# AnirudhKaushik10/Efficient-Workers-in-Distributed-Machine-Learning

Hardware: AMD Instinct MI355X
Metric: grad bytes/step on wire + images/sec, VGG-11 CIFAR-10 at 1/2/4/8 MI355X (higher is better)
Workload: dtype fp32

## Files before the change

efficient-workers-in-distributed-machine-learning_amd/ops/csrc/bindings.cpp:

```cpp
#include <pybind11/pybind11.h>
#include <pybind11/stl.h>

#include <vector>

#include "ewdml_ops.h"

namespace py = pybind11;
using Ptrs = std::vector<uintptr_t>;
using Mask = std::vector<uint32_t>;

static GradSrc grad_src(const Ptrs& grads, const Mask& mask) {
  return GradSrc{grads.data(), (int)grads.size(), mask.data(), (int)mask.size()};
}

template <class A, void (*fn)(const A&)>
static void with_grads(A a, const Ptrs& grads, const Mask& mask) {
  a.src = grad_src(grads, mask);
  fn(a);
}

static StepArgs default_step() {
  StepArgs s{};
  s.grad_scale = 1.0f;
  return s;
// ... 233 lines not shown
  m.def("cf_flush_wgout", &ew_cf_flush_wgout);
  m.def("bn_part_floats", &ew_bn_part_floats);
  m.def("bn_relu_fwd",
        [](uintptr_t h, uintptr_t res, uintptr_t y, uintptr_t code, uintptr_t stats,
           uintptr_t part, uintptr_t gamma, uintptr_t beta, uintptr_t cbias, uintptr_t rmean,
           uintptr_t rvar, uintptr_t nbt, long long N, int H, int W, int C, int is_bf16,
           int pool, int mode, int training, float momentum, float eps, int cb_bf16,
           uintptr_t stream, int pre_nblk, int phase) {
          BnFwdArgs a{};
          a.pre_nblk = pre_nblk;
          a.phase = phase;
          a.h = h; a.res = res; a.y = y; a.code = code; a.stats = stats; a.part = part;
          a.gamma = gamma; a.beta = beta; a.cbias = cbias; a.rmean = rmean; a.rvar = rvar;
          a.nbt = nbt; a.N = N; a.H = H; a.W = W; a.C = C;
          a.is_bf16 = is_bf16; a.pool = pool; a.mode = mode; a.training = training;
          a.momentum = momentum; a.eps = eps; a.cb_bf16 = cb_bf16; a.stream = stream;
          ew_bn_relu_fwd(a);
        });
  m.def("bn_relu_bwd",
        [](uintptr_t h, uintptr_t res, uintptr_t dy, uintptr_t code, uintptr_t stats,
           uintptr_t coef, uintptr_t part, uintptr_t dx, uintptr_t dres, uintptr_t dgamma,
           uintptr_t dbeta, uintptr_t dcbias, long long N, int H, int W, int C, int is_bf16,
           int pool, int mode, int cb_bf16, uintptr_t stream, int pre_nblk, int phase) {
          BnBwdArgs a{};
          a.phase = phase;
          a.h = h; a.res = res; a.dy = dy; a.code = code; a.stats = stats; a.coef = coef;
          a.part = part; a.dx = dx; a.dres = dres; a.dgamma = dgamma; a.dbeta = dbeta;
          a.dcbias = dcbias; a.N = N; a.H = H; a.W = W; a.C = C; a.is_bf16 = is_bf16;
          a.pool = pool; a.mode = mode; a.cb_bf16 = cb_bf16; a.stream = stream;
          a.pre_nblk = pre_nblk;
          ew_bn_relu_bwd(a);
        });
  m.def("act_dropout_fwd", &ew_act_dropout_fwd);
  m.def("act_dropout_bwd", &ew_act_dropout_bwd);
  m.def("cross_entropy_fwd", &ew_cross_entropy_fwd);
  m.def("cross_entropy_bwd", &ew_cross_entropy_bwd);
  m.def("conv_ws_floats", &ew_conv_ws_floats);
  m.def("conv_fwd", &ew_conv_fwd);
  m.def("conv_bwd_data", &ew_conv_bwd_data);
  m.def("conv_wgrad", &ew_conv_wgrad);
  m.def("conv_stem_fwd", &ew_conv_stem_fwd);
  m.def("head_fwd", &ew_head_fwd);
  m.def("head_fwd_ce", &ew_head_fwd_ce);
  m.def("head_bwd", &ew_head_bwd);
  m.def("head_bwd_bn", &ew_head_bwd_bn);
  m.def("conv_stem_wgrad", &ew_conv_stem_wgrad);
  m.def("rccl_unique_id", [] { return pybind11::bytes(ew_rccl_unique_id()); });
  m.def("rccl_version", &ew_rccl_version);
  m.def("rccl_init", [](pybind11::bytes uid, int nranks, int rank, int device) {
    return ew_rccl_init(std::string(uid), nranks, rank, device);
  });
  m.def("rccl_destroy", &ew_rccl_destroy);
  m.def("rccl_abort", &ew_rccl_abort);
  m.def("rccl_watchdog_start", &ew_rccl_watchdog_start);
  m.def("rccl_watch", &ew_rccl_watch);
  m.def("rccl_watch_pending", &ew_rccl_watch_pending);
  m.def("rccl_watchdog_stop", &ew_rccl_watchdog_stop,
        pybind11::call_guard<pybind11::gil_scoped_release>());
  m.def("test_flag_alloc", &ew_test_flag_alloc);
  m.def("test_flag_free", &ew_test_flag_free);
  m.def("watchdog_release_flag", &ew_watchdog_release_flag);
  m.def("test_spin", &ew_test_spin);
  m.def("rccl_all_gather", &ew_rccl_all_gather);
  m.def("rccl_all_reduce", &ew_rccl_all_reduce);
  m.def("rccl_reduce_scatter", &ew_rccl_reduce_scatter);
  m.def("rccl_broadcast", &ew_rccl_broadcast);
  m.def("rccl_all_to_all", &ew_rccl_all_to_all);
  m.def("conv_f32_fwd", &ew_conv_f32_fwd);
  m.def("conv_f32_bwd_data", &ew_conv_f32_bwd_data);
  m.def("conv_f32_wgrad", &ew_conv_f32_wgrad);
  m.def("conv_f32_fwd_lz", &ew_conv_f32_fwd_lz);
  m.def("conv_f32_wgrad_lz", &ew_conv_f32_wgrad_lz);
  m.def("conv_f32_fwd_s2", &ew_conv_f32_fwd_s2);
  m.def("conv_f32_bwd_data_s2", &ew_conv_f32_bwd_data_s2);
  m.def("conv_f32_wgrad_s2", &ew_conv_f32_wgrad_s2);
  m.def("conv_f32_stem_fwd", &ew_conv_f32_stem_fwd);
  m.def("conv_f32_stem_wgrad", &ew_conv_f32_stem_wgrad);
  m.def("conv_f32_stem_wgrad_bn", &ew_conv_f32_stem_wgrad_bn);
  m.def("wino_f32_weight", &ew_wino_f32_weight);
  m.def("wino_f32_fwd", &ew_wino_f32_fwd);
  m.def("wino_f32_bwd_data", &ew_wino_f32_bwd_data);
  m.def("wino_f32_wgrad", &ew_wino_f32_wgrad);
  m.def("wino_f32_wgrad_out", &ew_wino_f32_wgrad_out);
  m.def("wino_f32_fwd_bn", &ew_wino_f32_fwd_bn);
  m.def("wino_f32_bwd_data_bn", &ew_wino_f32_bwd_data_bn);
  m.def("sm_f32_ws_floats", &ew_sm_f32_ws_floats);
  m.def("sm_f32_counters", &ew_sm_f32_counters);
  m.def("sm_f32_fwd", &ew_sm_f32_fwd);
  m.def("sm_set_fence", &ew_sm_set_fence);
  m.def("topk_fused_select_max_blocks", &ew_topk_fused_select_max_blocks);
  m.def("topk_one_max_blocks", &ew_topk_one_max_blocks);
  m.def("flag_signal", &ew_flag_signal);
  m.def("flag_wait", &ew_flag_wait);
  m.def("topk_one_stamps", &ew_topk_one_stamps);
  m.def("sm_f32_bwd", &ew_sm_f32_bwd);
  m.def("lenet_ws_floats", &ew_lenet_ws_floats);
  m.def("lenet_counters", &ew_lenet_counters);
  m.def("lenet_set_prof", &ew_lenet_set_prof);
  m.def("lenet_fwd", &ew_lenet_fwd);
  m.def("tail_ws_floats", &ew_tail_ws_floats);
  m.def("tail_counters", &ew_tail_counters);
  m.def("tail_fwd", &ew_tail_fwd);
  m.def("tail_bwd", &ew_tail_bwd);
  m.def("lenet_bwd", &ew_lenet_bwd);
  m.def("maxpool2_nhwc", &ew_maxpool2_nhwc);
  m.def("maxpool3s2_nhwc", &ew_maxpool3s2_nhwc);
  m.def("gap_nhwc", &ew_gap_nhwc);
  m.def("maxpool2_fwd", &ew_maxpool2_fwd);
  m.def("maxpool2_bwd", &ew_maxpool2_bwd);
  m.def("ticket_ints", [] { return EW_TICKET_INTS; });
  m.def("make_batch",
        [](uintptr_t src, uintptr_t labels, uintptr_t perm, long long perm_len, uintptr_t state,
           uintptr_t done, uintptr_t out, uintptr_t out_y, int B, int C, int H, int W, int pad, int augment,
           int out_bf16, int channels_last, uint32_t seed, uint32_t rank,
           const std::vector<float>& mean, const std::vector<float>& inv_std, uintptr_t stream) {
          MakeBatchArgs a{};
          a.src = src; a.labels = labels; a.perm = perm; a.perm_len = perm_len; a.state = state; a.done = done;
          a.out = out; a.out_y = out_y; a.B = B; a.C = C; a.H = H; a.W = W; a.pad = pad;
          a.augment = augment; a.out_bf16 = out_bf16; a.channels_last = channels_last;
          a.seed = seed; a.rank = rank;
          for (int c = 0; c < 4; ++c) {
            a.mean[c] = c < (int)mean.size() ? mean[c] : 0.0f;
            a.inv_std[c] = c < (int)inv_std.size() ? inv_std[c] : 1.0f;
          }
          a.stream = stream;
          ew_make_batch(a);
        });
}
```

efficient-workers-in-distributed-machine-learning_amd/ops/csrc/ewdml_ops.h:

```cpp
#pragma once
#include <stdexcept>
#include <string>
#include <vector>
#include <stddef.h>
#include <stdint.h>

struct GradSrc {
  const uintptr_t* grad_ptrs;
  int n_grad_ptrs;
  const uint32_t* bf16_mask;
  int n_bf16_mask;
};

struct StepArgs {
  uintptr_t param, mom, grad_out, shadow;
  float lr, momentum, dampening, weight_decay, grad_scale;
  int nesterov, first, apply;
  uintptr_t key_state;
  uint32_t key_seed, key_rank;
  uintptr_t lr_ptr;
};

inline void ew_step_check(const std::string& who, const StepArgs& s, bool need_mom) {
  if (s.apply && !s.param) throw std::runtime_error(who + ": apply needs the parameters");
// ... 467 lines not shown
void ew_head_fwd(uintptr_t x, uintptr_t w, uintptr_t b, uintptr_t z, uintptr_t y, int B, int N,
                 int K, int relu, uintptr_t ctr_in, uint32_t salt_in, float p_in,
                 uintptr_t ctr_out, uint32_t salt_out, float p_out, uintptr_t stream,
                 int is_f32);
void ew_head_fwd_ce(uintptr_t x, uintptr_t w, uintptr_t b, uintptr_t z, int B, int N, int K,
                    uintptr_t yl, uintptr_t lossrow, uintptr_t loss, uintptr_t lse, uintptr_t dlog,
                    uintptr_t tick, uintptr_t stream, int is_f32);
void ew_head_bwd_bn(uintptr_t dz, uintptr_t y, uintptr_t x, uintptr_t w, uintptr_t dx,
                    uintptr_t dw, uintptr_t db, int B, int N, int K, int relu, uintptr_t ctr_out,
                    uint32_t salt_out, float p_out, uintptr_t ctr_in, uint32_t salt_in,
                    float p_in, int advance, uintptr_t bn_h, uintptr_t bn_code,
                    uintptr_t bn_stats, uintptr_t bn_coef, uintptr_t bn_dgamma,
                    uintptr_t bn_dbeta, uintptr_t bn_dcbias, int bn_cb_bf16, uintptr_t bn_tick,
                    uintptr_t stream);
void ew_head_bwd(uintptr_t dz, uintptr_t y, uintptr_t x, uintptr_t w, uintptr_t dx, uintptr_t dw,
                 uintptr_t db, int db_bf16, int B, int N, int K, int relu, uintptr_t ctr_out,
                 uint32_t salt_out, float p_out, uintptr_t ctr_in, uint32_t salt_in, float p_in,
                 int advance, uintptr_t stream, int is_f32);
int ew_conv_stem_fwd(uintptr_t x, uintptr_t w, uintptr_t y, long long N, int H, int W, int Nc,
                     uintptr_t bnpart, long long bnpart_floats, uintptr_t stream);
void ew_conv_stem_wgrad(uintptr_t dy, uintptr_t x, uintptr_t dw, uintptr_t ws,
                        long long ws_floats, long long N, int H, int W, int Nc, uintptr_t stream);

int ew_conv_f32_fwd(uintptr_t x, uintptr_t w, uintptr_t y, uintptr_t ws, long long ws_floats,
                    long long N, int H, int W, int C, int Nc, int ksize, uintptr_t bnpart,
                    long long bnpart_floats, uintptr_t stream);
int ew_conv_f32_bwd_data(uintptr_t dy, uintptr_t w, uintptr_t dx, uintptr_t ws,
                         long long ws_floats, long long N, int H, int W, int C, int Nc, int ksize,
                         uintptr_t bn_h, uintptr_t bn_res, uintptr_t bn_code, uintptr_t bn_stats,
                         int bn_relu, uintptr_t bnpart, long long bnpart_floats, uintptr_t addend,
                         uintptr_t stream);
void ew_conv_f32_wgrad(uintptr_t dy, uintptr_t x, uintptr_t dw, uintptr_t ws, long long ws_floats,
                       long long N, int H, int W, int C, int Nc, int ksize, uintptr_t stream);
int ew_conv_f32_fwd_lz(uintptr_t h, uintptr_t stats, uintptr_t nbt, uintptr_t w, uintptr_t y,
                       uintptr_t ws, long long ws_floats, long long N, int H, int W, int C, int Nc,
                       uintptr_t bnpart, long long bnpart_floats, uintptr_t stream);
void ew_conv_f32_wgrad_lz(uintptr_t dy, uintptr_t h, uintptr_t stats, uintptr_t dw, uintptr_t ws,
                          long long ws_floats, long long N, int H, int W, int C, int Nc,
                          uintptr_t stream);
int ew_conv_f32_fwd_s2(uintptr_t x, uintptr_t w, uintptr_t y, uintptr_t ws, long long ws_floats,
                       long long N, int H, int W, int C, int Nc, int ksize, uintptr_t bnpart,
                       long long bnpart_floats, uintptr_t stream);
void ew_conv_f32_bwd_data_s2(uintptr_t dy, uintptr_t w, uintptr_t dx, long long N, int H, int W,
                             int C, int Nc, int ksize, uintptr_t addend, uintptr_t stream);
void ew_conv_f32_wgrad_s2(uintptr_t dy, uintptr_t x, uintptr_t dw, uintptr_t ws,
                          long long ws_floats, long long N, int H, int W, int C, int Nc, int ksize,
                          uintptr_t stream);
int ew_conv_f32_stem_fwd(uintptr_t x, uintptr_t w, uintptr_t y, long long N, int H, int W, int Nc,
                         uintptr_t bnpart, long long bnpart_floats, uintptr_t stream);
void ew_conv_f32_stem_wgrad(uintptr_t dy, uintptr_t x, uintptr_t dw, uintptr_t ws,
                            long long ws_floats, long long N, int H, int W, int Nc,
                            uintptr_t stream);
void ew_conv_f32_stem_wgrad_bn(uintptr_t h, uintptr_t dnext, uintptr_t code, uintptr_t stats,
                               uintptr_t coef, int pool, uintptr_t x, uintptr_t dw, uintptr_t ws,
                               long long ws_floats, long long N, int H, int W, int Nc,
                               uintptr_t stream);
void ew_wino_f32_weight(uintptr_t w, uintptr_t U, int Nc, int C, int m, uintptr_t stream);
int ew_wino_f32_fwd(uintptr_t x, uintptr_t w, uintptr_t U, uintptr_t y, uintptr_t V, uintptr_t Mo,
                    long long N, int H, int W, int C, int Nc, int m, uintptr_t bnpart,
                    long long bnpart_floats, uintptr_t stream);
int ew_wino_f32_bwd_data(uintptr_t dy, uintptr_t w, uintptr_t U, uintptr_t dx, uintptr_t V,
                         uintptr_t Mo, long long N, int H, int W, int C, int Nc, int m,
                         uintptr_t bn_h, uintptr_t bn_res, uintptr_t bn_code, uintptr_t bn_stats,
                         int bn_relu, uintptr_t bnpart, long long bnpart_floats,
                         uintptr_t addend, uintptr_t D, uintptr_t wo_src, int wo_split,
                         uintptr_t wo_dw, int wo_Nc, int wo_C, uintptr_t stream);
int ew_wino_f32_fwd_bn(uintptr_t bn_h, uintptr_t bn_stats, uintptr_t bn_code, uintptr_t nbt,
                       int pool, uintptr_t w, uintptr_t U, uintptr_t y, uintptr_t V,
                       uintptr_t Mo, long long N, int H, int W, int C, int Nc, int m,
                       uintptr_t bnpart, long long bnpart_floats, uintptr_t stream);
int ew_wino_f32_bwd_data_bn(uintptr_t out_h, uintptr_t out_dnext, uintptr_t out_code,
                            uintptr_t out_stats, uintptr_t out_coef, int out_pool, uintptr_t w,
                            uintptr_t U, uintptr_t dx, uintptr_t V, uintptr_t Mo, long long N,
                            int H, int W, int C, int Nc, int m, uintptr_t bn_h, uintptr_t bn_res,
                            uintptr_t bn_code, uintptr_t bn_stats, int bn_relu, uintptr_t bnpart,
                            long long bnpart_floats, uintptr_t addend, uintptr_t D,
                            uintptr_t wo_src, int wo_split, uintptr_t wo_dw, int wo_Nc, int wo_C,
                            uintptr_t stream);
int ew_wino_f32_wgrad(uintptr_t dy, uintptr_t V, uintptr_t dw, uintptr_t D, int d_ready,
                      uintptr_t U_scratch, uintptr_t ws, long long ws_floats, long long N, int H,
                      int W, int C, int Nc, int m, int defer_out, uintptr_t stream);
void ew_wino_f32_wgrad_out(uintptr_t src, int split, uintptr_t dw, int Nc, int C, int m,
                           uintptr_t stream);

long long ew_sm_f32_ws_floats(long long N, int C, int Nc);
int ew_sm_set_fence(int on);
long long ew_sm_f32_counters(long long N, int C, int Nc);
int ew_sm_f32_fwd(uintptr_t x, uintptr_t bn_h, uintptr_t bn_stats, uintptr_t nbt, uintptr_t w,
                  uintptr_t y, uintptr_t slab, long long slab_floats, uintptr_t cnt,
                  long long cnt_ints, long long N, int C, int Nc, uintptr_t bnpart,
                  long long bnpart_floats, uintptr_t stream);
int ew_sm_f32_bwd(uintptr_t x, uintptr_t bn_h, uintptr_t bn_stats, uintptr_t dy,
                  uintptr_t out_h, uintptr_t out_dnext, uintptr_t out_code, uintptr_t out_stats,
                  uintptr_t out_coef, int out_pool, uintptr_t w, uintptr_t dx, uintptr_t dw,
                  uintptr_t slab, long long slab_floats, uintptr_t cnt, long long cnt_ints,
                  long long N, int C, int Nc, uintptr_t pb_h, uintptr_t pb_res, uintptr_t pb_code,
                  uintptr_t pb_stats, int pb_relu, uintptr_t bnpart, long long bnpart_floats,
                  uintptr_t fin_coef, uintptr_t fin_dgamma, uintptr_t fin_dbeta,
                  uintptr_t fin_dcbias, int fin_cb_bf16, long long fin_M, uintptr_t stream,
                  uintptr_t st_vel = 0, uintptr_t st_resid = 0, uintptr_t st_param = 0,
                  float st_momentum = 0.0f, float st_damp1 = 1.0f, float st_wd = 0.0f,
                  int st_nesterov = 0, uintptr_t st_lr = 0, uintptr_t st_stamp = 0);

long long ew_lenet_ws_floats(int B);
int ew_lenet_counters(int B);
void ew_lenet_set_prof(uintptr_t buf);
void ew_lenet_fwd(uintptr_t x, uintptr_t w1, uintptr_t b1, uintptr_t w2, uintptr_t b2,
                  uintptr_t wf1, uintptr_t bf1, uintptr_t wf2, uintptr_t bf2, uintptr_t y, int B,
                  int K, uintptr_t a1, uintptr_t code1, uintptr_t a2, uintptr_t code2,
                  uintptr_t h1, uintptr_t logits, uintptr_t dlogits, uintptr_t dh1,
                  uintptr_t lossrow, uintptr_t loss, uintptr_t ws, long long ws_floats,
                  uintptr_t cnt, int cnt_ints, uintptr_t stream, uintptr_t bsrc = 0,
                  uintptr_t blabels = 0, uintptr_t bperm = 0, long long bperm_len = 0,
                  uintptr_t bstate = 0, uintptr_t bdone = 0, float bmean = 0.0f,
                  float binv_std = 1.0f);
void ew_lenet_bwd(uintptr_t x, uintptr_t w2, uintptr_t wf1, uintptr_t a1, uintptr_t code1,
                  uintptr_t a2, uintptr_t code2, uintptr_t h1, uintptr_t dlogits, uintptr_t dh1,
                  uintptr_t gscale, int B, int K, uintptr_t dp2, uintptr_t dw1, uintptr_t db1,
                  uintptr_t dw2, uintptr_t db2, uintptr_t dwf1, uintptr_t dbf1, uintptr_t dwf2,
                  uintptr_t dbf2, uintptr_t ws, long long ws_floats, uintptr_t cnt, int cnt_ints,
                  uintptr_t stream);

long long ew_tail_ws_floats(int B, int N2);
int ew_tail_counters(int B);
void ew_tail_fwd(uintptr_t h1, uintptr_t w2, uintptr_t b2, uintptr_t w3, uintptr_t b3, uintptr_t y,
                 int B, int K1, int N2, int K, uintptr_t h2, uintptr_t logits, uintptr_t dlogits,
                 uintptr_t dh2, uintptr_t lossrow, uintptr_t loss, uintptr_t ws,
                 long long ws_floats, uintptr_t cnt, int cnt_ints, uintptr_t stream);
void ew_tail_bwd(uintptr_t h1, uintptr_t h2, uintptr_t dh2, uintptr_t dlogits, uintptr_t w2,
                 uintptr_t gscale, int B, int K1, int N2, int K, uintptr_t dh1, uintptr_t dw2,
                 uintptr_t db2, uintptr_t dw3, uintptr_t db3, uintptr_t stream);

std::string ew_rccl_unique_id();
int ew_rccl_version();
uintptr_t ew_rccl_init(const std::string& uid, int nranks, int rank, int device);
void ew_rccl_destroy(uintptr_t h);
void ew_rccl_abort(uintptr_t h);
uintptr_t ew_rccl_watchdog_start(uintptr_t comm, int device, double timeout_s, int exit_code);
void ew_rccl_watch(uintptr_t wd, uintptr_t stream);
int ew_rccl_watch_pending(uintptr_t wd);
void ew_rccl_watchdog_stop(uintptr_t wd);
uintptr_t ew_test_flag_alloc();
void ew_test_flag_free(uintptr_t f);
void ew_watchdog_release_flag(uintptr_t wd, uintptr_t f);
void ew_test_spin(uintptr_t flag, double max_s, uintptr_t stream);
void ew_rccl_all_gather(uintptr_t h, uintptr_t send, uintptr_t recv, long long count, int dtype,
                        uintptr_t stream);
void ew_rccl_all_reduce(uintptr_t h, uintptr_t send, uintptr_t recv, long long count, int dtype,
                        int op, uintptr_t stream);
void ew_rccl_reduce_scatter(uintptr_t h, uintptr_t send, uintptr_t recv, long long count,
                            int dtype, int op, uintptr_t stream);
void ew_rccl_broadcast(uintptr_t h, uintptr_t send, uintptr_t recv, long long count, int dtype,
                       int root, uintptr_t stream);
void ew_rccl_all_to_all(uintptr_t h, uintptr_t send, uintptr_t recv, long long count, int dtype,
                        int nranks, uintptr_t stream);

void ew_cross_entropy_fwd(uintptr_t x, uintptr_t y, int B, int K, int is_bf16, uintptr_t loss,
                          uintptr_t lse, uintptr_t stream, uintptr_t dx);
void ew_cross_entropy_bwd(uintptr_t x, uintptr_t y, uintptr_t lse, uintptr_t grad, int B, int K,
                          int is_bf16, uintptr_t dx, uintptr_t stream);

void ew_act_dropout_fwd(uintptr_t y, uintptr_t z, int n, float p, int relu, uintptr_t ctr,
                        uint32_t salt, uintptr_t stream);
void ew_act_dropout_bwd(uintptr_t dz, uintptr_t y, uintptr_t dy, uintptr_t db, int db_bf16,
                        int rows, int C, float p, int relu, uintptr_t ctr, uint32_t salt,
                        uintptr_t stream);
// ... 1 lines not shown
```

efficient-workers-in-distributed-machine-learning_amd/ops/csrc/winograd_f32.hip:

```cpp
#include <stdexcept>
#include <string>

#include "common.h"
#include "conv_f32.h"
#include "wg_common.h"
#include "ewdml_ops.h"

int ew_cf_gemm_tn_batched(const float* a, const float* b, float* out, float* ws,
                          long long ws_floats, int M, int N, int K, int batch, long long a_bs,
                          long long b_bs, hipStream_t s);
void ew_cf_gemm_batched(const float* a, const float* b, float* out, int M, int N, int K, int batch,
                        long long a_bs, long long b_bs, long long o_bs, bool nt, bool flip,
                        hipStream_t s);

namespace {

template <int M, bool FLIP>
__device__ __forceinline__ void wg_weight(const float* __restrict__ w, float* __restrict__ U,
                                          int Nc, int C, long long g) {
  using T = typename Wg<M>::V;
  constexpr int A = Wg<M>::A, VW = Wg<M>::VW;
  const int cq = C / VW;
  if (g >= (long long)Nc * cq) return;
  const int o = (int)(g / cq), i = (int)(g - (long long)o * cq) * VW;
// ... 270 lines not shown
      for (int i = 0; i < M; ++i) u[i][b] = wg_dot<A>([&](int a) { return wg_at<M>(i, a); }, col);
    }
    const int n = (int)(tl / tpi), rem = (int)(tl - (long long)n * tpi);
    const int ty = rem / tw, tx = rem - ty * tw;
#pragma unroll
    for (int i = 0; i < M; ++i)
#pragma unroll
      for (int j = 0; j < M; ++j) {
        T v = wg_dot<A>([&](int b) { return wg_at<M>(j, b); }, u[i]);
        const long long r = ((long long)n * H + M * ty + i) * W + M * tx + j;
        const long long off = r * Nc + c0;
        if (addend) v += *reinterpret_cast<const T*>(addend + off);
        *reinterpret_cast<T*>(y + off) = v;
        if (!bnpart) continue;
        if (!bb.h) {
#pragma unroll
          for (int q = 0; q < VW; ++q) {
            s1[q] += v[q];
            s2[q] += v[q] * v[q];
          }
          continue;
        }
        T xh, rr{};
        if (bb.code) {
          const uint32_t p = (uint32_t)r, nn = p / HoWo, rm = p - nn * HoWo;
          const uint32_t ho = rm / (uint32_t)bb.Wo, wo = rm - ho * (uint32_t)bb.Wo;
          const uint32_t base = 4 * nn * HoWo + 4 * ho * (uint32_t)bb.Wo + 2 * wo;
          uint32_t kw;
          if constexpr (VW == 4)
            kw = *reinterpret_cast<const uint32_t*>(bb.code + off);
          else
            kw = *reinterpret_cast<const uint16_t*>(bb.code + off);
          T hq[4], rq[4];
#pragma unroll
          for (int qq = 0; qq < 4; ++qq) {
            const size_t hr = base + (qq >> 1) * (2 * (uint32_t)bb.Wo) + (qq & 1);
            hq[qq] = *reinterpret_cast<const T*>(bb.h + hr * Nc + c0);
            if (bb.res) rq[qq] = *reinterpret_cast<const T*>(bb.res + hr * Nc + c0);
          }
#pragma unroll
          for (int q = 0; q < VW; ++q) {
            const uint32_t k = (kw >> (8 * q)) & 3u;
            xh[q] = k == 0 ? hq[0][q] : k == 1 ? hq[1][q] : k == 2 ? hq[2][q] : hq[3][q];
            if (bb.res) rr[q] = k == 0 ? rq[0][q] : k == 1 ? rq[1][q] : k == 2 ? rq[2][q] : rq[3][q];
          }
        } else {
          xh = *reinterpret_cast<const T*>(bb.h + (size_t)r * Nc + c0);
          if (bb.res) rr = *reinterpret_cast<const T*>(bb.res + (size_t)r * Nc + c0);
        }
#pragma unroll
        for (int q = 0; q < VW; ++q) {
          float z = xh[q] * sc[q] + sh[q];
          if (bb.res) z = z + rr[q];
          const float dz = (bb.relu == 0 || !(z <= 0.0f)) ? v[q] : 0.0f;
          s1[q] += dz;
          s2[q] += dz * (xh[q] - mean[q]);
        }
      }
  }
  if (!bnpart) return;
  {
    T a, b;
#pragma unroll
    for (int q = 0; q < VW; ++q) {
      a[q] = s1[q];
      b[q] = s2[q];
    }
    *reinterpret_cast<T*>(&red[0][rg * Nc + c0]) = a;
    *reinterpret_cast<T*>(&red[1][rg * Nc + c0]) = b;
  }
  __syncthreads();
  const int nb = gridDim.x;
  for (int c = t; c < Nc; c += EW_BLOCK) {
    float a = 0.0f, q = 0.0f;
    for (int i = 0; i < rpi; ++i) {
      a += red[0][i * Nc + c];
      q += red[1][i * Nc + c];
    }
    bnpart[(long long)blockIdx.x * Nc + c] = a;
    bnpart[(long long)(nb + blockIdx.x) * Nc + c] = q;
  }
}


template <int M>
__global__ __launch_bounds__(EW_BLOCK) void k_wg_wgrad_out(const float* __restrict__ src,
                                                           int nsplit, float* __restrict__ dw,
                                                           int Nc, int C) {
  wg_wgrad_out<M>(src, nsplit, dw, Nc, C, (long long)blockIdx.x * EW_BLOCK + threadIdx.x);
}

long long wg_tiles(int m, long long N, int H, int W) { return N * (H / m) * (W / m); }

void wg_check(int m, long long N, int H, int W, int Cin, int Cout, const char* what) {
  const long long tiles = wg_tiles(m, N, H, W);
  const int vw = m == 2 ? WG2_VW : 2;
  const bool pow2 = Cout >= 64 && Cout <= 256 * vw && (Cout & (Cout - 1)) == 0;
  if ((m != 2 && m != 4) || H % m || W % m || tiles % 64 || Cin % 32 || !pow2 ||
      (long long)(m + 2) * (m + 2) * tiles * std::max(Cin, Cout) >= (1LL << 31))
    throw std::runtime_error(std::string("ewdml winograd f32 ") + what +
                             ": needs m in {2, 4}, H, W % m == 0, N*H*W/m^2 % 64 == 0, C_in % 32 "
                             "== 0, C_out a power of two in [64, 256 * (m == 2 ? 4 : 2)]");
}

template <int M>
int wg_output(const float* Mo, float* y, long long N, int H, int W, int Nc, float* bnpart,
              long long bnpart_floats, const CfBnBwd& bb, const float* addend, hipStream_t s) {
  const long long tiles = wg_tiles(M, N, H, W);
  const int ovw = Nc <= 2 * EW_BLOCK ? 2 : 4;
  const int rpi = EW_BLOCK / (Nc / ovw);
  long long tpb = rpi, nblk = (tiles + tpb - 1) / tpb;
  if (bnpart) {
    while (nblk > 1024) {
      tpb += rpi;
      nblk = (tiles + tpb - 1) / tpb;
    }
    if (2LL * nblk * Nc > bnpart_floats) bnpart = nullptr;
  }
  if (!bnpart) {
    tpb = rpi;
    nblk = (tiles + tpb - 1) / tpb;
  }
  if (ovw == 2)
    hipLaunchKernelGGL((k_wg_output<M, 2>), dim3((unsigned)nblk), dim3(EW_BLOCK), 0, s, Mo, y, H,
                       W, Nc, tiles, (int)tpb, bnpart, bb, addend);
  else
    hipLaunchKernelGGL((k_wg_output<M, 4>), dim3((unsigned)nblk), dim3(EW_BLOCK), 0, s, Mo, y, H,
                       W, Nc, tiles, (int)tpb, bnpart, bb, addend);
  EW_CHECK_LAUNCH();
  return bnpart ? (int)nblk : 0;
}

template <int M, bool FLIP>
void wg_input(const float* x, float* V, long long N, int H, int W, int C, hipStream_t s,
              const float* w, float* U, int Nw, int Cw, float* D, const WgSrc* src = nullptr,
              int kind = 0, const WgOut* rider = nullptr) {
  constexpr int VW = Wg<M>::VW;
  const long long n = wg_tiles(M, N, H, W) * (C / VW);
  const int nbi = (int)((n + EW_BLOCK - 1) / EW_BLOCK);
  const int nbw = w ? (int)(((long long)Nw * (Cw / VW) + EW_BLOCK - 1) / EW_BLOCK) : 0;
  const WgOut no_out{nullptr, nullptr, 1, 0, 0};
  const WgOut& wo = rider && rider->src ? *rider : no_out;
  const int nbo = wo.src ? (int)(((long long)wo.Nc * (wo.C / VW) + EW_BLOCK - 1) / EW_BLOCK) : 0;
  const WgSrc none{nullptr, nullptr, nullptr, nullptr, nullptr, nullptr, 0};
  const WgSrc& sr = src ? *src : none;
#define WG_IN(K_)                                                                                \
  hipLaunchKernelGGL((k_wg_input<M, FLIP, K_>), dim3(nbi + nbw + nbo), dim3(EW_BLOCK), 0, s, x, V, \
                     H, W, C, wg_tiles(M, N, H, W), nbi, w, U, Nw, Cw, D, sr, nbw, wo)
  if (kind == 1) WG_IN(1);
  else if (kind == 2) WG_IN(2);
  else WG_IN(0);
#undef WG_IN
  EW_CHECK_LAUNCH();
}

template <int M>
int wino_fwd(const float* x, const float* w, float* U, float* y, float* v, float* mo, long long N,
             int H, int W, int C, int Nc, float* bnpart, long long bnpart_floats, hipStream_t s,
             const WgSrc* src) {
  constexpr int AA = Wg<M>::A * Wg<M>::A;
  const long long tiles = wg_tiles(M, N, H, W);
  wg_input<M, false>(x, v, N, H, W, C, s, w, U, Nc, C, nullptr, src, src ? 1 : 0);
  ew_cf_gemm_batched(v, U, mo, (int)tiles, Nc, C, AA, tiles * C, (long long)Nc * C, tiles * Nc,
                     true, false, s);
  const CfBnBwd none{nullptr, nullptr, nullptr, nullptr, 0, 0, 0};
  return wg_output<M>(mo, y, N, H, W, Nc, bnpart, bnpart_floats, none, nullptr, s);
}

template <int M>
int wino_bwd(const float* dy, const float* w, float* U, float* dx, float* v, float* mo,
             long long N, int H, int W, int C, int Nc, const CfBnBwd& bb, float* bnpart,
             long long bnpart_floats, const float* addend, float* D, hipStream_t s,
             const WgSrc* src, const WgOut* rider) {
  const int kind = src ? 2 : 0;
  constexpr int AA = Wg<M>::A * Wg<M>::A;
  const long long tiles = wg_tiles(M, N, H, W);
  if constexpr (M == 4)
    wg_input<M, true>(dy, v, N, H, W, Nc, s, w, U, Nc, C, D, src, kind, rider);
  else
    wg_input<M, false>(dy, v, N, H, W, Nc, s, nullptr, nullptr, 0, 0, D, src, kind, rider);
  ew_cf_gemm_batched(v, U, mo, (int)tiles, C, Nc, AA, tiles * Nc, (long long)Nc * C, tiles * C,
                     false, M == 2, s);
  return wg_output<M>(mo, dx, N, H, W, C, bnpart, bnpart_floats, bb, addend, s);
}

template <int M>
int wino_wgrad(const float* dy, const float* V, float* dw, float* d, int d_ready, float* du,
               float* ws, long long ws_floats, long long N, int H, int W, int C, int Nc,
               int defer_out, hipStream_t s) {
  constexpr int A = Wg<M>::A, VW = Wg<M>::VW;
  const long long tiles = wg_tiles(M, N, H, W);
  if (!d_ready) {
    const long long n = tiles * (Nc / VW);
    hipLaunchKernelGGL(k_wg_dy<M>, dim3((unsigned)((n + EW_BLOCK - 1) / EW_BLOCK)),
                       dim3(EW_BLOCK), 0, s, dy, d, H, W, Nc, tiles);
    EW_CHECK_LAUNCH();
  }
  const int split = ew_cf_gemm_tn_batched(d, V, du, ws, ws_floats, Nc, C, (int)tiles, A * A,
                                          tiles * Nc, tiles * C, s);
  if (defer_out) return split;
  const long long m = (long long)Nc * (C / VW);
  hipLaunchKernelGGL(k_wg_wgrad_out<M>, dim3((unsigned)((m + EW_BLOCK - 1) / EW_BLOCK)),
                     dim3(EW_BLOCK), 0, s, split > 1 ? ws : du, split, dw, Nc, C);
  EW_CHECK_LAUNCH();
  return split;
}

}

void ew_wino_f32_weight(uintptr_t w, uintptr_t U, int Nc, int C, int m, uintptr_t stream) {
  const int vw = m == 2 ? WG2_VW : 2;
// ... 24 lines not shown
int ew_wino_f32_fwd_bn(uintptr_t bn_h, uintptr_t bn_stats, uintptr_t bn_code, uintptr_t nbt,
                       int pool, uintptr_t w, uintptr_t U, uintptr_t y, uintptr_t V,
                       uintptr_t Mo, long long N, int H, int W, int C, int Nc, int m,
                       uintptr_t bnpart, long long bnpart_floats, uintptr_t stream) {
  wg_check(m, N, H, W, C, Nc, "forward");
  if (pool && !bn_code) throw std::runtime_error("ewdml winograd f32: pooled input needs codes");
  const WgSrc src{reinterpret_cast<const float*>(bn_h), reinterpret_cast<const float*>(bn_stats),
                  reinterpret_cast<uint8_t*>(bn_code), nullptr, nullptr,
                  reinterpret_cast<long long*>(nbt), pool};
  auto* f = m == 2 ? wino_fwd<2> : wino_fwd<4>;
  return f(nullptr, reinterpret_cast<const float*>(w), reinterpret_cast<float*>(U),
           reinterpret_cast<float*>(y), reinterpret_cast<float*>(V), reinterpret_cast<float*>(Mo),
           N, H, W, C, Nc, reinterpret_cast<float*>(bnpart), bnpart_floats, (hipStream_t)stream,
           &src);
}

static WgOut wg_rider(uintptr_t src, int split, uintptr_t dw, int Nc, int C, int m) {
  const int vw = m == 2 ? WG2_VW : 2;
  if (src && (!dw || split < 1 || Nc <= 0 || C % vw))
    throw std::runtime_error("ewdml winograd f32: bad riding weight-gradient output transform");
  return WgOut{reinterpret_cast<const float*>(src), reinterpret_cast<float*>(dw), split, Nc, C};
}

int ew_wino_f32_bwd_data(uintptr_t dy, uintptr_t w, uintptr_t U, uintptr_t dx, uintptr_t V,
                         uintptr_t Mo, long long N, int H, int W, int C, int Nc, int m,
                         uintptr_t bn_h, uintptr_t bn_res, uintptr_t bn_code, uintptr_t bn_stats,
                         int bn_relu, uintptr_t bnpart, long long bnpart_floats,
                         uintptr_t addend, uintptr_t D, uintptr_t wo_src, int wo_split,
                         uintptr_t wo_dw, int wo_Nc, int wo_C, uintptr_t stream) {
  const WgOut rider = wg_rider(wo_src, wo_split, wo_dw, wo_Nc, wo_C, m);
  wg_check(m, N, H, W, Nc, C, "backward data");
  if (m == 4 && !w) throw std::runtime_error("ewdml winograd f32: m = 4 backward needs w");
  const CfBnBwd bb{reinterpret_cast<const float*>(bn_h), reinterpret_cast<const float*>(bn_res),
                   reinterpret_cast<const uint8_t*>(bn_code),
                   reinterpret_cast<const float*>(bn_stats), bn_relu, H, W};
  auto* f = m == 2 ? wino_bwd<2> : wino_bwd<4>;
  return f(reinterpret_cast<const float*>(dy), reinterpret_cast<const float*>(w),
           reinterpret_cast<float*>(U), reinterpret_cast<float*>(dx), reinterpret_cast<float*>(V),
           reinterpret_cast<float*>(Mo), N, H, W, C, Nc, bb,
           bn_h ? reinterpret_cast<float*>(bnpart) : nullptr, bnpart_floats,
           reinterpret_cast<const float*>(addend), reinterpret_cast<float*>(D),
           (hipStream_t)stream, nullptr, &rider);
}

int ew_wino_f32_bwd_data_bn(uintptr_t out_h, uintptr_t out_dnext, uintptr_t out_code,
                            uintptr_t out_stats, uintptr_t out_coef, int out_pool, uintptr_t w,
                            uintptr_t U, uintptr_t dx, uintptr_t V, uintptr_t Mo, long long N,
                            int H, int W, int C, int Nc, int m, uintptr_t bn_h, uintptr_t bn_res,
                            uintptr_t bn_code, uintptr_t bn_stats, int bn_relu, uintptr_t bnpart,
                            long long bnpart_floats, uintptr_t addend, uintptr_t D,
                            uintptr_t wo_src, int wo_split, uintptr_t wo_dw, int wo_Nc, int wo_C,
                            uintptr_t stream) {
  const WgOut rider = wg_rider(wo_src, wo_split, wo_dw, wo_Nc, wo_C, m);
  wg_check(m, N, H, W, Nc, C, "backward data");
  if (m == 4 && !w) throw std::runtime_error("ewdml winograd f32: m = 4 backward needs w");
  if (out_pool && (H % 2 || W % 2 || !out_code))
    throw std::runtime_error("ewdml winograd f32: pooled BN backward needs even maps and codes");
  const WgSrc src{reinterpret_cast<const float*>(out_h), reinterpret_cast<const float*>(out_stats),
                  reinterpret_cast<uint8_t*>(out_code), reinterpret_cast<const float*>(out_coef),
                  reinterpret_cast<const float*>(out_dnext), nullptr, out_pool};
  const CfBnBwd bb{reinterpret_cast<const float*>(bn_h), reinterpret_cast<const float*>(bn_res),
                   reinterpret_cast<const uint8_t*>(bn_code),
                   reinterpret_cast<const float*>(bn_stats), bn_relu, H, W};
  auto* f = m == 2 ? wino_bwd<2> : wino_bwd<4>;
  return f(nullptr, reinterpret_cast<const float*>(w), reinterpret_cast<float*>(U),
           reinterpret_cast<float*>(dx), reinterpret_cast<float*>(V), reinterpret_cast<float*>(Mo),
           N, H, W, C, Nc, bb, bn_h ? reinterpret_cast<float*>(bnpart) : nullptr, bnpart_floats,
           reinterpret_cast<const float*>(addend), reinterpret_cast<float*>(D),
           (hipStream_t)stream, &src, &rider);
}

int ew_wino_f32_wgrad(uintptr_t dy, uintptr_t V, uintptr_t dw, uintptr_t D, int d_ready,
                      uintptr_t U_scratch, uintptr_t ws, long long ws_floats, long long N, int H,
                      int W, int C, int Nc, int m, int defer_out, uintptr_t stream) {
  wg_check(m, N, H, W, C, Nc, "weight gradient");
  if (C % 64) throw std::runtime_error("ewdml winograd f32: weight gradient needs C % 64 == 0");
  auto* f = m == 2 ? wino_wgrad<2> : wino_wgrad<4>;
  return f(reinterpret_cast<const float*>(dy), reinterpret_cast<const float*>(V),
           reinterpret_cast<float*>(dw), reinterpret_cast<float*>(D), d_ready,
           reinterpret_cast<float*>(U_scratch), reinterpret_cast<float*>(ws), ws_floats, N, H, W,
           C, Nc, defer_out, (hipStream_t)stream);
}

void ew_wino_f32_wgrad_out(uintptr_t src, int split, uintptr_t dw, int Nc, int C, int m,
                           uintptr_t stream) {
  const WgOut wo = wg_rider(src, split, dw, Nc, C, m);
  if (!wo.src) return;
  const int vw = m == 2 ? WG2_VW : 2;
  const long long n = (long long)Nc * (C / vw);
  const dim3 grid((unsigned)((n + EW_BLOCK - 1) / EW_BLOCK));
  if (m == 2)
    hipLaunchKernelGGL(k_wg_wgrad_out<2>, grid, dim3(EW_BLOCK), 0, (hipStream_t)stream, wo.src,
                       wo.nsplit, wo.dw, Nc, C);
  else
    hipLaunchKernelGGL(k_wg_wgrad_out<4>, grid, dim3(EW_BLOCK), 0, (hipStream_t)stream, wo.src,
                       wo.nsplit, wo.dw, Nc, C);
  EW_CHECK_LAUNCH();
}
```

Measured before the change: 112,500.

## Add software-pipelined Winograd output transform kernel with specialized epilogues

Adds a Winograd output-transform kernel that double-buffers the transformed tiles in registers, prefetching the next tile while the current one is computed. The batch-norm, residual, ReLU and addend epilogues become compile-time template parameters. By default it is used only for the m=2, narrow-channel, non-residual cases, chosen through an environment variable, and it also exposes a direct output-transform binding and a mode setter. The aim is to hide global-load latency and remove runtime branching, at the cost of higher register pressure and several template instantiations.

```diff
diff --git a/efficient-workers-in-distributed-machine-learning_amd/ops/csrc/bindings.cpp b/efficient-workers-in-distributed-machine-learning_amd/ops/csrc/bindings.cpp
--- a/efficient-workers-in-distributed-machine-learning_amd/ops/csrc/bindings.cpp
+++ b/efficient-workers-in-distributed-machine-learning_amd/ops/csrc/bindings.cpp
@@ -339,6 +339,8 @@
   m.def("wino_f32_bwd_data", &ew_wino_f32_bwd_data);
   m.def("wino_f32_wgrad", &ew_wino_f32_wgrad);
   m.def("wino_f32_wgrad_out", &ew_wino_f32_wgrad_out);
+  m.def("wino_f32_output", &ew_wino_f32_output);
+  m.def("wg_set_out_pipe", &ew_wg_set_out_pipe);
   m.def("wino_f32_fwd_bn", &ew_wino_f32_fwd_bn);
   m.def("wino_f32_bwd_data_bn", &ew_wino_f32_bwd_data_bn);
   m.def("sm_f32_ws_floats", &ew_sm_f32_ws_floats);
diff --git a/efficient-workers-in-distributed-machine-learning_amd/ops/csrc/ewdml_ops.h b/efficient-workers-in-distributed-machine-learning_amd/ops/csrc/ewdml_ops.h
--- a/efficient-workers-in-distributed-machine-learning_amd/ops/csrc/ewdml_ops.h
+++ b/efficient-workers-in-distributed-machine-learning_amd/ops/csrc/ewdml_ops.h
@@ -573,6 +573,11 @@
                       int W, int C, int Nc, int m, int defer_out, uintptr_t stream);
 void ew_wino_f32_wgrad_out(uintptr_t src, int split, uintptr_t dw, int Nc, int C, int m,
                            uintptr_t stream);
+int ew_wino_f32_output(uintptr_t Mo, uintptr_t y, long long N, int H, int W, int Nc, int m,
+                       uintptr_t bn_h, uintptr_t bn_res, uintptr_t bn_code, uintptr_t bn_stats,
+                       int bn_relu, uintptr_t bnpart, long long bnpart_floats, uintptr_t addend,
+                       int tpb, uintptr_t stream);
+int ew_wg_set_out_pipe(int on);
 
 long long ew_sm_f32_ws_floats(long long N, int C, int Nc);
 int ew_sm_set_fence(int on);
diff --git a/efficient-workers-in-distributed-machine-learning_amd/ops/csrc/winograd_f32.hip b/efficient-workers-in-distributed-machine-learning_amd/ops/csrc/winograd_f32.hip
--- a/efficient-workers-in-distributed-machine-learning_amd/ops/csrc/winograd_f32.hip
+++ b/efficient-workers-in-distributed-machine-learning_amd/ops/csrc/winograd_f32.hip
@@ -376,6 +376,170 @@
   }
 }
 
+enum { WO_NONE = 0, WO_FWD = 1, WO_BWD = 2, WO_BWDC = 3 };
+
+template <int M, int VW, int STAT, bool RES, bool RELU, bool ADD>
+__global__ __launch_bounds__(EW_BLOCK) void k_wg_output_p(const float* __restrict__ Mo,
+                                                          float* __restrict__ y, int H, int W,
+                                                          int Nc, long long tiles, int tpb,
+                                                          float* __restrict__ bnpart, CfBnBwd bb,
+                                                          const float* __restrict__ addend) {
+  typedef float T __attribute__((ext_vector_type(VW)));
+  constexpr int A = Wg<M>::A;
+  constexpr bool BWD = STAT == WO_BWD || STAT == WO_BWDC;
+  constexpr int NQ = STAT == WO_BWDC ? 4 : 1;
+  constexpr int ER = M == 4 ? 1 : M;
+  static_assert(BWD || (!RES && !RELU), "res / relu belong to the backward sums");
+  __shared__ __attribute__((aligned(16))) float red[2][EW_BLOCK * 4];
+  const int tpr = Nc / VW, rpi = EW_BLOCK / tpr;
+  const int t = threadIdx.x, rg = t / tpr, c0 = (t - rg * tpr) * VW;
+  const long long t0 = (long long)blockIdx.x * tpb;
+  const long long t1 = t0 + tpb < tiles ? t0 + tpb : tiles;
+  const int tw = W / M, tpi = (H / M) * tw;
+  const long long xs = tiles * Nc;
+  const uint32_t HoWo = (uint32_t)bb.Ho * bb.Wo;
+  float s1[VW], s2[VW], mean[VW], sc[VW], sh[VW];
+#pragma unroll
+  for (int j = 0; j < VW; ++j) s1[j] = s2[j] = 0.0f;
+  if constexpr (BWD) {
+#pragma unroll
+    for (int j = 0; j < VW; ++j) {
+      mean[j] = bb.stats[c0 + j];
+      sc[j] = bb.stats[2 * Nc + c0 + j];
+      sh[j] = bb.stats[3 * Nc + c0 + j];
+    }
+  }
+  auto load_mo = [&](T (&mo)[A][A], long long tile) __attribute__((always_inline)) {
+    const uint32_t bo = ((uint32_t)tile * (uint32_t)Nc + (uint32_t)c0) * 4u;
+#pragma unroll
+    for (int b = 0; b < A; ++b)
+#pragma unroll
+      for (int a = 0; a < A; ++a)
+        mo[b][a] = *reinterpret_cast<const T*>(reinterpret_cast<const char*>(Mo + (a * A + b) * xs) + bo);
+  };
+  auto step = [&](long long tl, const T (&cur)[A][A], T (&nxt)[A][A]) __attribute__((always_inline)) {
+    const bool more = tl + rpi < t1;
+    if (more) load_mo(nxt, tl + rpi);
+    const int n = (int)((uint32_t)tl / (uint32_t)tpi), rem = (int)tl - n * tpi;
+    const int ty = rem / tw, tx = rem - ty * tw;
+    T u[M][A];
+#pragma unroll
+    for (int i0 = 0; i0 < M; i0 += ER) {
+      T ad[ER][M], hq[ER][M][NQ], rq[ER][M][NQ];
+      uint32_t kw[ER][M];
+#pragma unroll
+      for (int ii = 0; ii < ER; ++ii)
+#pragma unroll
+        for (int j = 0; j < M; ++j) {
+          const long long r = ((long long)n * H + M * ty + i0 + ii) * W + M * tx + j;
+          const long long off = r * Nc + c0;
+          if constexpr (ADD) ad[ii][j] = *reinterpret_cast<const T*>(addend + off);
+          if constexpr (STAT == WO_BWDC) {
+            const uint32_t p = (uint32_t)r, nn = p / HoWo, rm = p - nn * HoWo;
+            const uint32_t ho = rm / (uint32_t)bb.Wo, wo = rm - ho * (uint32_t)bb.Wo;
+            const uint32_t base = 4 * nn * HoWo + 4 * ho * (uint32_t)bb.Wo + 2 * wo;
+            if constexpr (VW == 4)
+              kw[ii][j] = *reinterpret_cast<const uint32_t*>(bb.code + off);
+            else
+              kw[ii][j] = *reinterpret_cast<const uint16_t*>(bb.code + off);
+#pragma unroll
+            for (int qq = 0; qq < 4; ++qq) {
+              const size_t hr = base + (qq >> 1) * (2 * (uint32_t)bb.Wo) + (qq & 1);
+              hq[ii][j][qq] = *reinterpret_cast<const T*>(bb.h + hr * Nc + c0);
+              if constexpr (RES) rq[ii][j][qq] = *reinterpret_cast<const T*>(bb.res + hr * Nc + c0);
+            }
+          } else if constexpr (STAT == WO_BWD) {
+            hq[ii][j][0] = *reinterpret_cast<const T*>(bb.h + (size_t)r * Nc + c0);
+            if constexpr (RES) rq[ii][j][0] = *reinterpret_cast<const T*>(bb.res + (size_t)r * Nc + c0);
+          }
+        }
+      if (i0 == 0) {
+#pragma unroll
+        for (int b = 0; b < A; ++b)
+#pragma unroll
+          for (int i = 0; i < M; ++i)
+            u[i][b] = wg_dot<A>([&](int a) { return wg_at<M>(i, a); }, cur[b]);
+      }
+#pragma unroll
+      for (int ii = 0; ii < ER; ++ii)
+#pragma unroll
+        for (int j = 0; j < M; ++j) {
+          const int i = i0 + ii;
+          T v = wg_dot<A>([&](int b) { return wg_at<M>(j, b); }, u[i]);
+          const long long r = ((long long)n * H + M * ty + i) * W + M * tx + j;
+          const long long off = r * Nc + c0;
+          if constexpr (ADD) v += ad[ii][j];
+          *reinterpret_cast<T*>(y + off) = v;
+          if constexpr (STAT == WO_FWD) {
+#pragma unroll
+            for (int q = 0; q < VW; ++q) {
+              s1[q] += v[q];
+              s2[q] += v[q] * v[q];
+            }
+          }
+          if constexpr (BWD) {
+            T xh, rr{};
+            if constexpr (STAT == WO_BWDC) {
+#pragma unroll
+              for (int q = 0; q < VW; ++q) {
+                const uint32_t k = (kw[ii][j] >> (8 * q)) & 3u;
+                const T(&hh)[4] = hq[ii][j];
+                xh[q] = k == 0 ? hh[0][q] : k == 1 ? hh[1][q] : k == 2 ? hh[2][q] : hh[3][q];
+                if constexpr (RES) {
+                  const T(&rs)[4] = rq[ii][j];
+                  rr[q] = k == 0 ? rs[0][q] : k == 1 ? rs[1][q] : k == 2 ? rs[2][q] : rs[3][q];
+                }
+              }
+            } else {
+              xh = hq[ii][j][0];
+              if constexpr (RES) rr = rq[ii][j][0];
+            }
+#pragma unroll
+            for (int q = 0; q < VW; ++q) {
+              float z = xh[q] * sc[q] + sh[q];
+              if constexpr (RES) z = z + rr[q];
+              const float dz = (!RELU || !(z <= 0.0f)) ? v[q] : 0.0f;
+              s1[q] += dz;
+              s2[q] += dz * (xh[q] - mean[q]);
+            }
+          }
+        }
+    }
+    return more;
+  };
+  long long tl = t0 + rg;
+  if (tl < t1) {
+    T ra[A][A], rb[A][A];
+    load_mo(ra, tl);
+    for (;; tl += 2 * rpi) {
+      if (!step(tl, ra, rb)) break;
+      if (!step(tl + rpi, rb, ra)) break;
+    }
+  }
+  if constexpr (STAT == WO_NONE) return;
+  {
+    T a, b;
+#pragma unroll
+    for (int q = 0; q < VW; ++q) {
+      a[q] = s1[q];
+      b[q] = s2[q];
+    }
+    *reinterpret_cast<T*>(&red[0][rg * Nc + c0]) = a;
+    *reinterpret_cast<T*>(&red[1][rg * Nc + c0]) = b;
+  }
+  __syncthreads();
+  const int nb = gridDim.x;
+  for (int c = t; c < Nc; c += EW_BLOCK) {
+    float a = 0.0f, q = 0.0f;
+    for (int i = 0; i < rpi; ++i) {
+      a += red[0][i * Nc + c];
+      q += red[1][i * Nc + c];
+    }
+    bnpart[(long long)blockIdx.x * Nc + c] = a;
+    bnpart[(long long)(nb + blockIdx.x) * Nc + c] = q;
+  }
+}
+
 
 template <int M>
 __global__ __launch_bounds__(EW_BLOCK) void k_wg_wgrad_out(const float* __restrict__ src,
@@ -397,30 +561,101 @@
                              "== 0, C_out a power of two in [64, 256 * (m == 2 ? 4 : 2)]");
 }
 
+int g_wg_out_pipe = -1;
+int wg_out_pipe_mode() {
+  if (g_wg_out_pipe < 0) {
+    const char* e = getenv("EWDML_WG_OUT_PIPE");
+    g_wg_out_pipe = (e && e[0] == '0') ? 0 : (e && e[0] == '1') ? 1 : 2;
+  }
+  return g_wg_out_pipe;
+}
+
+template <int M, int VW>
+void wg_output_p(int stat, bool res, bool relu, bool add, dim3 grid, hipStream_t s,
+                 const float* Mo, float* y, int H, int W, int Nc, long long tiles, int tpb,
+                 float* bnpart, const CfBnBwd& bb, const float* addend) {
+#define WO_CASE(S_, RES_, RELU_, ADD_)                                                          \
+  if (stat == S_ && res == RES_ && relu == RELU_ && add == ADD_) {                              \
+    hipLaunchKernelGGL((k_wg_output_p<M, VW, S_, RES_, RELU_, ADD_>), grid, dim3(EW_BLOCK), 0, s, \
+                       Mo, y, H, W, Nc, tiles, tpb, bnpart, bb, addend);                        \
+    return;                                                                                     \
+  }
+  WO_CASE(WO_NONE, false, false, false)
+  WO_CASE(WO_NONE, false, false, true)
+  WO_CASE(WO_FWD, false, false, false)
+  WO_CASE(WO_BWD, false, false, false)
+  WO_CASE(WO_BWD, false, false, true)
+  WO_CASE(WO_BWD, false, true, false)
+  WO_CASE(WO_BWD, false, true, true)
+  WO_CASE(WO_BWD, true, false, false)
+  WO_CASE(WO_BWD, true, false, true)
+  WO_CASE(WO_BWD, true, true, false)
+  WO_CASE(WO_BWD, true, true, true)
+  WO_CASE(WO_BWDC, false, false, false)
+  WO_CASE(WO_BWDC, false, true, false)
+#undef WO_CASE
+  throw std::runtime_error(
+      "ewdml winograd f32 output transform: no pipelined kernel for this epilogue (statistics " +
+      std::to_string(stat) + ", residual " + std::to_string((int)res) + ", relu " +
+      std::to_string((int)relu) + ", addend " + std::to_string((int)add) +
+      "); EWDML_WG_OUT_PIPE=0 or 2 runs the general kernel");
+}
+
+bool wg_out_pipe_measured(int m, int ovw, int stat, bool res, bool relu, bool add) {
+  return m == 2 && ovw == 2 && !res && !add &&
+         (stat == WO_FWD || ((stat == WO_BWD || stat == WO_BWDC) && relu));
+}
+
 template <int M>
 int wg_output(const float* Mo, float* y, long long N, int H, int W, int Nc, float* bnpart,
-              long long bnpart_floats, const CfBnBwd& bb, const float* addend, hipStream_t s) {
+              long long bnpart_floats, const CfBnBwd& bb, const float* addend, hipStream_t s,
+              int tpb_force = 0) {
   const long long tiles = wg_tiles(M, N, H, W);
   const int ovw = Nc <= 2 * EW_BLOCK ? 2 : 4;
   const int rpi = EW_BLOCK / (Nc / ovw);
   long long tpb = rpi, nblk = (tiles + tpb - 1) / tpb;
-  if (bnpart) {
-    while (nblk > 1024) {
-      tpb += rpi;
+  if (tpb_force > 0) {
+    tpb = tpb_force;
+    nblk = (tiles + tpb - 1) / tpb;
+    if (bnpart && 2LL * nblk * Nc > bnpart_floats)
+      throw std::runtime_error("ewdml winograd f32 output transform: bnpart too small");
+  } else {
+    if (bnpart) {
+      while (nblk > 1024) {
+        tpb += rpi;
+        nblk = (tiles + tpb - 1) / tpb;
+      }
+      if (2LL * nblk * Nc > bnpart_floats) bnpart = nullptr;
+    }
+    if (!bnpart) {
+      tpb = rpi;
       nblk = (tiles + tpb - 1) / tpb;
     }
-    if (2LL * nblk * Nc > bnpart_floats) bnpart = nullptr;
-  }
-  if (!bnpart) {
-    tpb = rpi;
-    nblk = (tiles + tpb - 1) / tpb;
-  }
-  if (ovw == 2)
+  }
+  const int stat = !bnpart ? WO_NONE : !bb.h ? WO_FWD : bb.code ? WO_BWDC : WO_BWD;
+  const bool bwd = stat == WO_BWD || stat == WO_BWDC;
+  const bool res = bwd && bb.res, relu = bwd && bb.relu != 0;
+  const int pipe = wg_out_pipe_mode();
+  if (pipe == 1 || (pipe == 2 && wg_out_pipe_measured(M, ovw, stat, res, relu, addend != nullptr))) {
+    if (tiles * Nc >= (1LL << 30))
+      throw std::runtime_error("ewdml winograd f32 output transform: the pipelined kernel needs "
+                               "tiles * C_out < 2^30");
+    if (ovw == 2)
+      wg_output_p<M, 2>(stat, res, relu, addend != nullptr, dim3((unsigned)nblk), s, Mo, y, H, W,
+                        Nc, tiles, (int)tpb, bnpart, bb, addend);
+    else if constexpr (M == 2)
+      wg_output_p<M, 4>(stat, res, relu, addend != nullptr, dim3((unsigned)nblk), s, Mo, y, H, W,
+                        Nc, tiles, (int)tpb, bnpart, bb, addend);
+    else
+      throw std::runtime_error("ewdml winograd f32 output transform: no pipelined kernel for "
+                               "m = 4 with more than 512 output channels");
+  } else if (ovw == 2) {
     hipLaunchKernelGGL((k_wg_output<M, 2>), dim3((unsigned)nblk), dim3(EW_BLOCK), 0, s, Mo, y, H,
                        W, Nc, tiles, (int)tpb, bnpart, bb, addend);
-  else
+  } else {
     hipLaunchKernelGGL((k_wg_output<M, 4>), dim3((unsigned)nblk), dim3(EW_BLOCK), 0, s, Mo, y, H,
                        W, Nc, tiles, (int)tpb, bnpart, bb, addend);
+  }
   EW_CHECK_LAUNCH();
   return bnpart ? (int)nblk : 0;
 }
@@ -611,6 +846,35 @@
            C, Nc, defer_out, (hipStream_t)stream);
 }
 
+int ew_wg_set_out_pipe(int on) {
+  const int prev = wg_out_pipe_mode();
+  if (on >= 0) g_wg_out_pipe = on > 2 ? 2 : on;
+  return prev;
+}
+
+int ew_wino_f32_output(uintptr_t Mo, uintptr_t y, long long N, int H, int W, int Nc, int m,
+                       uintptr_t bn_h, uintptr_t bn_res, uintptr_t bn_code, uintptr_t bn_stats,
+                       int bn_relu, uintptr_t bnpart, long long bnpart_floats, uintptr_t addend,
+                       int tpb, uintptr_t stream) {
+  const bool pow2 = Nc >= 64 && Nc <= 4 * EW_BLOCK && (Nc & (Nc - 1)) == 0;
+  if ((m != 2 && m != 4) || N <= 0 || H <= 0 || W <= 0 || H % m || W % m || !pow2 || tpb < 0 ||
+      !Mo || !y || (bn_h && !bn_stats) || ((bn_res || bn_code) && !bn_h) ||
+      (long long)N * H * W >= (1LL << 29) ||
+      (long long)(m + 2) * (m + 2) * wg_tiles(m, N, H, W) * Nc >= (1LL << 31))
+    throw std::runtime_error("ewdml winograd f32 output transform: needs m in {2, 4}, H, W % m "
+                             "== 0, C_out a power of two in [64, 1024], Mo < 2^31 floats, stats with h");
+  const long long tiles = wg_tiles(m, N, H, W);
+  if (tpb > 0 && (tiles + tpb - 1) / tpb > 65535)
+    throw std::runtime_error("ewdml winograd f32 output transform: tpb too small");
+  const CfBnBwd bb{reinterpret_cast<const float*>(bn_h), reinterpret_cast<const float*>(bn_res),
+                   reinterpret_cast<const uint8_t*>(bn_code),
+                   reinterpret_cast<const float*>(bn_stats), bn_relu, H, W};
+  auto* f = m == 2 ? wg_output<2> : wg_output<4>;
+  return f(reinterpret_cast<const float*>(Mo), reinterpret_cast<float*>(y), N, H, W, Nc,
+           reinterpret_cast<float*>(bnpart), bnpart_floats, bb,
+           reinterpret_cast<const float*>(addend), (hipStream_t)stream, tpb);
+}
+
 void ew_wino_f32_wgrad_out(uintptr_t src, int split, uintptr_t dw, int Nc, int C, int m,
                            uintptr_t stream) {
   const WgOut wo = wg_rider(src, split, dw, Nc, C, m);
```

After: 114,000, median of 6. 1.01x the previous value.
